# declare-lab/tango

Hardware: NVIDIA H100
Metric: audio_seconds_per_second (higher is better)
Workload: dtype bf16

## Files before the change

tango_b200/csrc/gemm_tc.cu:

```cuda
#include "tng_ptx.cuh"
#include "tng_internal.h"

namespace tng {

constexpr int BM = 128;
constexpr int BK = 64;
constexpr int A_TILE_BYTES = BM * BK * 2;
constexpr int GEMM_THREADS = 384;
constexpr int EPI_WARPS = 8;
constexpr int ES = 4;

struct KGroupDev {
  int view, a_c0, dw, dh, b_k0, nkb;
};

struct GemmKernelParams {
  int W, H, NB;
  int bw, bh, bn;
  int tiles_w, tiles_h, tiles_n;
  int m_tiles, n_tiles;
  int Ncols;
  int n_groups, total_kiters;
  int ksplit;
  KGroupDev g[TNG_MAX_KGROUPS];
  const float* bias;
  const float* rowvec;
  long long rowvec_ld;
  const void* res;
  int res_bf16;
  long long ldr;
  float alpha;
  int accumulate;
  float* out_f32;
  long long ld_f32;
  __nv_bfloat16* out_bf16;
  long long ld_bf16;
  int act;
  float act_param;
  int split_off;
  int fast_epi;
  double* col_stats;
  long long stats_hw;
};

template <int BN>
struct GemmCfg {
  static constexpr int B_TILE_BYTES = BN * BK * 2;
  static constexpr int STAGE_BYTES = A_TILE_BYTES + B_TILE_BYTES;
  static constexpr int EPI_BYTES = EPI_WARPS * 16 * 32 * 4;
  static constexpr int STAGES_RAW = (227 * 1024 - EPI_BYTES - 256) / STAGE_BYTES;
  static constexpr int STAGES = STAGES_RAW > 8 ? 8 : STAGES_RAW;
  static constexpr int SMEM_BYTES = STAGES * STAGE_BYTES + EPI_BYTES + 256 ;
};

enum EpiShape { EPI_SCALAR, EPI_VEC, EPI_FULL };

__device__ __forceinline__ float4 add4(float4 a, float4 b) { return make_float4(a.x + b.x, a.y + b.y, a.z + b.z, a.w + b.w); }
__device__ __forceinline__ float4 scale4(float4 a, float s) { return make_float4(a.x * s, a.y * s, a.z * s, a.w * s); }

template <int ACT>
__device__ __forceinline__ void act_chunk(float4 (&a)[ES], float ap) {
#pragma unroll
  for (int i = 0; i < ES; ++i)
    a[i] = make_float4(act_f(a[i].x, ACT, ap), act_f(a[i].y, ACT, ap), act_f(a[i].z, ACT, ap), act_f(a[i].w, ACT, ap));
}

__device__ __forceinline__ float4 staged(const float* st, int r, int cg) {
  return *reinterpret_cast<const float4*>(st + r * 32 + ((cg ^ (r & 7)) << 2));
}

template <bool VEC, bool RO = false, typename T>
__device__ __forceinline__ float4 load4(const T* q, int n) {
  if constexpr (VEC && sizeof(T) == 2) return load_bf16x4(q);
  if constexpr (VEC && sizeof(T) == 4)
    return RO ? __ldg(reinterpret_cast<const float4*>(q)) : *reinterpret_cast<const float4*>(q);
  float t[4] = {0.f, 0.f, 0.f, 0.f};
#pragma unroll
  for (int j = 0; j < 4; ++j)
    if (j < n) t[j] = static_cast<float>(RO ? __ldg(q + j) : q[j]);
  return make_float4(t[0], t[1], t[2], t[3]);
}

template <bool VEC>
__device__ __forceinline__ float4 load_bias(const GemmKernelParams& p, int col, int n) {
  return p.bias ? load4<VEC, true>(p.bias + col, n) : make_float4(0.f, 0.f, 0.f, 0.f);
}

template <bool VEC>
__device__ __forceinline__ float4 load_res(const GemmKernelParams& p, long long off, int n) {
  return p.res_bf16 ? load4<VEC>(static_cast<const __nv_bfloat16*>(p.res) + off, n)
                    : load4<VEC>(static_cast<const float*>(p.res) + off, n);
}

__device__ __forceinline__ void epi_stage(float* st, int lane, const float* v) {
  const int r = lane >> 2, t = lane & 3;
#pragma unroll
  for (int jj = 0; jj < 4; ++jj) {
    const int col = 8 * jj + 2 * t;
    const int off = (((col >> 2) ^ (r & 7)) << 2) + (col & 3);
    *reinterpret_cast<float2*>(st + r * 32 + off) = make_float2(v[4 * jj], v[4 * jj + 1]);
    *reinterpret_cast<float2*>(st + (r + 8) * 32 + off) = make_float2(v[4 * jj + 2], v[4 * jj + 3]);
  }
}

template <int BN>
__device__ __forceinline__ void stage_chunk(float* st, int lane, const float (&acc)[BN / 2], int c) {
  __syncwarp();
#pragma unroll
  for (int cc = 0; cc < BN / 32; ++cc)
    if (cc == c) epi_stage(st, lane, acc + 16 * cc);
  __syncwarp();
}

struct EpiTile {
  long long row_base;
  int n0, nvalid, tn, sp;
};

template <int BN, int SHAPE, int MODE>
__device__ __forceinline__ void epi_tile(const GemmKernelParams& p, float* st, const float (&acc)[BN / 2], const EpiTile& t,
                                         int wr, int lane) {
  constexpr bool FULL = SHAPE == EPI_FULL, VEC = SHAPE != EPI_SCALAR;
  const int cg = lane & 7, rsub = lane >> 3;
  const int trow = wr + rsub;
  const long long r0 = t.row_base + trow;
  const int lane_rows = FULL ? ES : min(ES, max(0, (t.nvalid - trow + 3) >> 2));
  const bool red = SHAPE == EPI_VEC && p.ksplit > 1;
  const bool add_terms = !red || t.sp == 0;
  const bool has_res = (MODE & 1) && (FULL || p.res) && add_terms;
  const bool has_f32 = (MODE & 2) && (FULL || p.out_f32);
  const bool has_bf = (MODE & 4) && (FULL || p.out_bf16);
  const bool has_rv = p.rowvec && add_terms;
  const int rpi = p.bw * p.bh;
  const int rpi_log2 = __ffs(rpi) - 1;
  const long long simg = (FULL && p.col_stats) ? (t.row_base + wr) / p.stats_hw : 0;
  const float4 zero = make_float4(0.f, 0.f, 0.f, 0.f);
#pragma unroll 1
  for (int c = 0; c < BN / 32; ++c) {
    stage_chunk<BN>(st, lane, acc, c);
    const int col = t.tn * BN + 32 * c + 4 * cg;
    const int ncols = FULL ? 4 : min(4, p.Ncols - col);
    const int nrows = ncols > 0 ? lane_rows : 0;
    float4 res[ES];
    if (has_res) {
      const long long off = r0 * p.ldr + col, rs = 4 * p.ldr;
#pragma unroll
      for (int i = 0; i < ES; ++i) res[i] = i < nrows ? load_res<VEC>(p, off + i * rs, ncols) : zero;
    }
    const float4 b4 = (add_terms && ncols > 0) ? load_bias<VEC>(p, col, ncols) : zero;
    float4 a[ES];
#pragma unroll
    for (int i = 0; i < ES; ++i) a[i] = add4(staged(st, 4 * i + rsub, cg), b4);
    if (has_rv) {
      float4 rv = zero;
#pragma unroll
      for (int i = 0; i < ES; ++i) {
        if (i >= nrows) continue;
        const long long img = t.n0 + ((trow + 4 * i) >> rpi_log2);
        if (i == 0 || rpi % 16 != 0) rv = load4<VEC, true>(p.rowvec + img * p.rowvec_ld + col, ncols);
        a[i] = add4(a[i], rv);
      }
    }
#pragma unroll
    for (int i = 0; i < ES; ++i) a[i] = scale4(has_res ? add4(a[i], res[i]) : a[i], p.alpha);
    if (has_f32) {
      float* op = p.out_f32 + r0 * p.ld_f32 + col;
      const long long os = 4 * p.ld_f32;
      if (p.accumulate) {
#pragma unroll
        for (int i = 0; i < ES; ++i)
          if (i < nrows) a[i] = add4(a[i], load4<VEC>(op + i * os, ncols));
      }
#pragma unroll
      for (int i = 0; i < ES; ++i) {
        if (i >= nrows) continue;
        float* q = op + i * os;
        if (red) {
          atomicAdd(q, a[i].x); atomicAdd(q + 1, a[i].y); atomicAdd(q + 2, a[i].z); atomicAdd(q + 3, a[i].w);
        } else if (VEC) {
          *reinterpret_cast<float4*>(q) = a[i];
        } else {
          const float v[4] = {a[i].x, a[i].y, a[i].z, a[i].w};
#pragma unroll
          for (int j = 0; j < 4; ++j)
            if (j < ncols) q[j] = v[j];
        }
      }
    }
    if (FULL && p.col_stats) {
      float s0 = 0.f, s1 = 0.f, s2 = 0.f, s3 = 0.f, q0 = 0.f, q1 = 0.f, q2 = 0.f, q3 = 0.f;
#pragma unroll
      for (int i = 0; i < ES; ++i) {
        s0 += a[i].x; s1 += a[i].y; s2 += a[i].z; s3 += a[i].w;
        q0 = fmaf(a[i].x, a[i].x, q0); q1 = fmaf(a[i].y, a[i].y, q1);
        q2 = fmaf(a[i].z, a[i].z, q2); q3 = fmaf(a[i].w, a[i].w, q3);
      }
#pragma unroll
      for (int o = 8; o <= 16; o <<= 1) {
        s0 += __shfl_xor_sync(0xffffffffu, s0, o); s1 += __shfl_xor_sync(0xffffffffu, s1, o);
        s2 += __shfl_xor_sync(0xffffffffu, s2, o); s3 += __shfl_xor_sync(0xffffffffu, s3, o);
        q0 += __shfl_xor_sync(0xffffffffu, q0, o); q1 += __shfl_xor_sync(0xffffffffu, q1, o);
        q2 += __shfl_xor_sync(0xffffffffu, q2, o); q3 += __shfl_xor_sync(0xffffffffu, q3, o);
      }
      if (rsub == 0) {
        double* sp = p.col_stats + (simg * p.Ncols + col) * 2;
        atomicAdd(sp + 0, static_cast<double>(s0)); atomicAdd(sp + 1, static_cast<double>(q0));
        atomicAdd(sp + 2, static_cast<double>(s1)); atomicAdd(sp + 3, static_cast<double>(q1));
        atomicAdd(sp + 4, static_cast<double>(s2)); atomicAdd(sp + 5, static_cast<double>(q2));
        atomicAdd(sp + 6, static_cast<double>(s3)); atomicAdd(sp + 7, static_cast<double>(q3));
      }
    }
    if (has_bf) {
      if (p.act == TNG_ACT_SILU) act_chunk<TNG_ACT_SILU>(a, p.act_param);
      else if (p.act == TNG_ACT_LRELU) act_chunk<TNG_ACT_LRELU>(a, p.act_param);
      __nv_bfloat16* op = p.out_bf16 + r0 * p.ld_bf16 + col;
      const long long os = 4 * p.ld_bf16;
#pragma unroll
      for (int i = 0; i < ES; ++i) {
        if (i >= nrows) continue;
        if (VEC) {
          store4_bf16(op + i * os, a[i]);
        } else {
          const float v[4] = {a[i].x, a[i].y, a[i].z, a[i].w};
#pragma unroll
          for (int j = 0; j < 4; ++j)
            if (j < ncols) store_bf16_split(op + i * os + j, v[j], p.split_off);
        }
      }
      if (VEC && p.split_off > 0) {
#pragma unroll
        for (int i = 0; i < ES; ++i)
          if (i < nrows) store4_bf16_lo(op + p.split_off + i * os, a[i]);
      }
    }
  }
}

template <int BN, bool FULL, bool SPLIT, bool TANH>
__device__ __forceinline__ void epi_tile_geglu(const GemmKernelParams& p, float* st, const float (&acc)[BN / 2],
                                               const EpiTile& t, int wr, int lane) {
  constexpr int HALF = BN / 2;
  const int cg = lane & 7, rsub = lane >> 3;
  const int trow = wr + rsub;
#pragma unroll 1
  for (int c = 0; c < HALF / 32; ++c) {
    float4 hid[ES], g[ES];
    stage_chunk<BN>(st, lane, acc, c);
#pragma unroll
    for (int i = 0; i < ES; ++i) hid[i] = staged(st, 4 * i + rsub, cg);
    stage_chunk<BN>(st, lane, acc, c + HALF / 32);
#pragma unroll
    for (int i = 0; i < ES; ++i) g[i] = staged(st, 4 * i + rsub, cg);
    const int gcol = t.tn * BN + 32 * c + 4 * cg;
    const int ocol = t.tn * HALF + 32 * c + 4 * cg;
    const float4 bh = load_bias<true>(p, gcol, 4), bg = load_bias<true>(p, gcol + HALF, 4);
#pragma unroll
    for (int i = 0; i < ES; ++i) {
      hid[i].x = (hid[i].x + bh.x) * (TANH ? gelu_tanh_f(g[i].x + bg.x) : gelu_erf_f(g[i].x + bg.x));
      hid[i].y = (hid[i].y + bh.y) * (TANH ? gelu_tanh_f(g[i].y + bg.y) : gelu_erf_f(g[i].y + bg.y));
      hid[i].z = (hid[i].z + bh.z) * (TANH ? gelu_tanh_f(g[i].z + bg.z) : gelu_erf_f(g[i].z + bg.z));
      hid[i].w = (hid[i].w + bh.w) * (TANH ? gelu_tanh_f(g[i].w + bg.w) : gelu_erf_f(g[i].w + bg.w));
    }
    __nv_bfloat16* op = p.out_bf16 + (t.row_base + trow) * p.ld_bf16 + ocol;
    const long long os = 4 * p.ld_bf16;
#pragma unroll
    for (int i = 0; i < ES; ++i) {
      if (!FULL && trow + 4 * i >= t.nvalid) continue;
      store4_bf16(op + i * os, hid[i]);
      if (SPLIT) store4_bf16_lo(op + p.split_off + i * os, hid[i]);
    }
  }
}

struct WorkItem {
  int sp, tn, w0, h0, n0;
};
__device__ __forceinline__ WorkItem work_item(const GemmKernelParams& p, int tile) {
  const int t2 = tile / p.ksplit, tm = t2 / p.n_tiles;
  const int tw = tm % p.tiles_w, th = (tm / p.tiles_w) % p.tiles_h, tb = tm / (p.tiles_w * p.tiles_h);
  return WorkItem{tile % p.ksplit, t2 % p.n_tiles, tw * p.bw, th * p.bh, tb * p.bn};
}

__device__ __forceinline__ int tile_kiters(const GemmKernelParams& p, int tile) {
  const int sp = tile % p.ksplit;
  return (sp + 1) * p.total_kiters / p.ksplit - sp * p.total_kiters / p.ksplit;
}

template <int BN>
__global__ void __launch_bounds__(GEMM_THREADS, 1)
gemm_tc_kernel(const __grid_constant__ CUtensorMap amap0, const __grid_constant__ CUtensorMap amap1,
               const __grid_constant__ CUtensorMap amap2, const __grid_constant__ CUtensorMap amap3,
               const __grid_constant__ CUtensorMap bmap, const __grid_constant__ GemmKernelParams p) {
  using Cfg = GemmCfg<BN>;
  constexpr int STAGES = Cfg::STAGES;
  extern __shared__ __align__(1024) uint8_t smem[];
  uint8_t* sA = smem;
  uint8_t* sB = smem + STAGES * A_TILE_BYTES;
  float* sEpi = reinterpret_cast<float*>(smem + STAGES * Cfg::STAGE_BYTES);
  uint64_t* full_bar = reinterpret_cast<uint64_t*>(smem + STAGES * Cfg::STAGE_BYTES + Cfg::EPI_BYTES);
  uint64_t* empty_bar = full_bar + STAGES;

  const int tid = threadIdx.x;
  const int warp = tid >> 5;
  const int lane = tid & 31;
  const int wg = warp >> 2;

  if (tid == 0) {
    if ((smem_u32(smem) & 1023u) != 0) __trap();
    tma_prefetch_desc(&amap0);
    tma_prefetch_desc(&bmap);
    for (int s = 0; s < STAGES; ++s) {
      mbar_init(&full_bar[s], 1);
      mbar_init(&empty_bar[s], 2);
    }
    fence_mbar_init();
  }
  __syncthreads();

  const int total_tiles = p.m_tiles * p.n_tiles * p.ksplit;
  const int work0 = blockIdx.x, work_stride = gridDim.x;

  if (wg == 0) {
    setmaxnreg_dec<40>();
    if (tid == 0) {
      uint32_t n_loaded = 0;
      for (int tile = work0; tile < total_tiles; tile += work_stride) {
        const WorkItem w = work_item(p, tile);
        const int nk = tile_kiters(p, tile);
        int k = w.sp * p.total_kiters / p.ksplit, gi = 0;
        while (k >= p.g[gi].nkb) { k -= p.g[gi].nkb; ++gi; }
        for (int ki = 0; ki < nk; ++ki, ++k, ++n_loaded) {
          if (k == p.g[gi].nkb) { k = 0; ++gi; }
          const int slot = static_cast<int>(n_loaded % STAGES);
          const uint32_t use = n_loaded / STAGES;
          if (use > 0) mbar_wait(&empty_bar[slot], (use - 1) & 1);
          const KGroupDev g = p.g[gi];
          const CUtensorMap* am = g.view == 0 ? &amap0 : g.view == 1 ? &amap1 : g.view == 2 ? &amap2 : &amap3;
          mbar_arrive_expect_tx(&full_bar[slot], Cfg::STAGE_BYTES);
          tma_load_4d(sA + slot * A_TILE_BYTES, am, &full_bar[slot], g.a_c0 + k * BK, w.w0 + g.dw, w.h0 + g.dh, w.n0);
          tma_load_2d(sB + slot * Cfg::B_TILE_BYTES, &bmap, &full_bar[slot], g.b_k0 + k * BK, w.tn * BN);
        }
      }
    }
    return;
  }
  setmaxnreg_inc<232>();

  const int cw = warp - 4;
  float* st = sEpi + cw * (16 * 32);
  const int wr = 16 * cw;
  const uint32_t a_off = static_cast<uint32_t>(wg - 1) * (64 * 128);
  const bool release = (tid & 127) == 0;
  const int mode = (p.res ? 1 : 0) | (p.out_f32 ? 2 : 0) | (p.out_bf16 ? 4 : 0);
  const bool geglu = (p.act == TNG_ACT_GEGLU || p.act == TNG_ACT_GEGLU_TANH);
  uint32_t n_used = 0;
  float acc[BN / 2];
#pragma unroll
  for (int i = 0; i < BN / 2; ++i) acc[i] = 0.f;
  for (int tile = work0; tile < total_tiles; tile += work_stride) {
    const int nk = tile_kiters(p, tile);
    for (int ki = 0; ki < nk; ++ki) {
      const int slot = static_cast<int>(n_used % STAGES);
      mbar_wait(&full_bar[slot], (n_used / STAGES) & 1);
      const uint64_t ad = wgmma_desc_sw128(smem_u32(sA + slot * A_TILE_BYTES) + a_off, 16, 1024);
      const uint64_t bd = wgmma_desc_sw128(smem_u32(sB + slot * Cfg::B_TILE_BYTES), 16, 1024);
      fence_regs(acc);
      wgmma_fence();
#pragma unroll
      for (int k = 0; k < BK / 16; ++k) wgmma_ss<BN>(acc, ad + 2 * k, bd + 2 * k, (ki > 0 || k > 0) ? 1u : 0u);
      wgmma_commit();
      fence_regs(acc);
      if (ki > 0) {
        wgmma_wait<1>();
        fence_regs(acc);
        mbar_arrive_if(&empty_bar[(n_used - 1) % STAGES], release);
      }
      ++n_used;
    }
    wgmma_wait<0>();
    fence_regs(acc);
    mbar_arrive_if(&empty_bar[(n_used - 1) % STAGES], release);

    const WorkItem w = work_item(p, tile);
    int nvalid;
    if (p.bh == 1 && p.bn == 1) nvalid = min(BM, p.W - w.w0);
    else if (p.bn == 1) nvalid = min(p.bh, p.H - w.h0) * p.bw;
    else nvalid = min(p.bn, p.NB - w.n0) * p.bh * p.bw;
    const EpiTile t{(static_cast<long long>(w.n0) * p.H + w.h0) * p.W + w.w0, w.n0, nvalid, w.tn, w.sp};
    if (geglu) {
      if constexpr (BN == 128 || BN == 256) {
        if (p.act == TNG_ACT_GEGLU_TANH) {
          if (p.split_off > 0) epi_tile_geglu<BN, false, true, true>(p, st, acc, t, wr, lane);
          else epi_tile_geglu<BN, false, false, true>(p, st, acc, t, wr, lane);
        } else if (p.split_off > 0) epi_tile_geglu<BN, false, true, false>(p, st, acc, t, wr, lane);
        else if (nvalid == BM) epi_tile_geglu<BN, true, false, false>(p, st, acc, t, wr, lane);
        else epi_tile_geglu<BN, false, false, false>(p, st, acc, t, wr, lane);
      }
    } else if (p.fast_epi && p.ksplit == 1 && nvalid == BM && (w.tn + 1) * BN <= p.Ncols) {
      switch (mode) {
        case 2: epi_tile<BN, EPI_FULL, 2>(p, st, acc, t, wr, lane); break;
        case 3: epi_tile<BN, EPI_FULL, 3>(p, st, acc, t, wr, lane); break;
        case 4: epi_tile<BN, EPI_FULL, 4>(p, st, acc, t, wr, lane); break;
        case 5: epi_tile<BN, EPI_FULL, 5>(p, st, acc, t, wr, lane); break;
        case 6: epi_tile<BN, EPI_FULL, 6>(p, st, acc, t, wr, lane); break;
        default: epi_tile<BN, EPI_FULL, 7>(p, st, acc, t, wr, lane); break;
      }
    } else if (p.fast_epi) {
      epi_tile<BN, EPI_VEC, 7>(p, st, acc, t, wr, lane);
    } else {
      epi_tile<BN, EPI_SCALAR, 7>(p, st, acc, t, wr, lane);
    }
  }
}

template <int BN>
static int launch_gemm(const CUtensorMap* am, const CUtensorMap& bm, const GemmKernelParams& p, cudaStream_t st) {
  using Cfg = GemmCfg<BN>;
  const int rc = set_max_dynamic_smem<gemm_tc_kernel<BN>>(Cfg::SMEM_BYTES, "gemm_tc");
  if (rc) return rc;
  const int work = p.m_tiles * p.n_tiles * p.ksplit;
  const int grid = work < num_sms() ? work : num_sms();
  gemm_tc_kernel<BN><<<grid, GEMM_THREADS, Cfg::SMEM_BYTES, st>>>(am[0], am[1], am[2], am[3], bm, p);
  return check_launch("gemm_tc");
}

static bool is_pow2(long long x) { return x > 0 && (x & (x - 1)) == 0; }

}

using namespace tng;

static int plan_gemm(const tng_gemm_desc* d, GemmKernelParams& p, int& bn_tile_out, bool& stats_after_out) {
  if (!d) return set_error(TNG_EINVAL, "null desc");
  if (d->n_aviews < 1 || d->n_aviews > TNG_MAX_AVIEWS) return set_error(TNG_EINVAL, "n_aviews=%d", d->n_aviews);
  if (d->n_groups < 1 || d->n_groups > TNG_MAX_KGROUPS) return set_error(TNG_EINVAL, "n_groups=%d", d->n_groups);
  if (d->W <= 0 || d->H <= 0 || d->NB <= 0 || d->Ncols <= 0) return set_error(TNG_EINVAL, "bad output grid");
  if ((d->ldb > 0 ? d->ldb : d->Ktot) % 8 != 0)
    return set_error(TNG_EINVAL, "B row stride must be a multiple of 8 elements (Ktot=%lld ldb=%lld)", (long long)d->Ktot, (long long)d->ldb);

  memset(&p, 0, sizeof(p));
  p.W = d->W; p.H = d->H; p.NB = d->NB;
  if (d->W >= BM || d->H == 1) {
    p.bw = BM; p.bh = 1; p.bn = 1;
  } else {
    if (!is_pow2(d->W)) return set_error(TNG_EINVAL, "W=%d < 128 must be a power of two", d->W);
    p.bw = d->W;
    const int rem = BM / p.bw;
    if (d->H >= rem) {
      p.bh = rem; p.bn = 1;
    } else {
      if (!is_pow2(d->H)) return set_error(TNG_EINVAL, "H=%d (W=%d) must be a power of two when W*H < 128", d->H, d->W);
      p.bh = d->H; p.bn = rem / p.bh;
    }
  }
  p.tiles_w = (d->W + p.bw - 1) / p.bw;
  p.tiles_h = (d->H + p.bh - 1) / p.bh;
  p.tiles_n = (d->NB + p.bn - 1) / p.bn;
  p.m_tiles = p.tiles_w * p.tiles_h * p.tiles_n;
  p.Ncols = (int)d->Ncols;

  int bn_tile = d->block_n;
  int ksplit = 1;
  if (d->act == TNG_ACT_GEGLU || d->act == TNG_ACT_GEGLU_TANH) {
    if (bn_tile == 0) bn_tile = (d->Ncols % 256 == 0) ? 256 : 128;
    if ((bn_tile != 128 && bn_tile != 256) || d->Ncols % bn_tile != 0 || !d->out_bf16 || d->out_f32 || d->res ||
        d->rowvec)
      return set_error(TNG_EINVAL, "GEGLU epilogue needs block_n 128/256 dividing Ncols, bf16 output only");
    if (d->alpha != 1.0f) return set_error(TNG_EINVAL, "GEGLU epilogue needs alpha = 1 (alpha=%g)", (double)d->alpha);
  }
  if (bn_tile == 0) {
    const long long N = d->Ncols;
    if (N <= 32) bn_tile = 32;
    else if (N <= 64) bn_tile = 64;
    else if (N % 256 == 0 && (long long)p.m_tiles * (N / 256) >= 2 * num_sms()) bn_tile = 256;
    else if (N % 160 == 0) {
      bn_tile = 160;
      if ((long long)p.m_tiles * (N / 160) * 2 <= num_sms()) {
        long long kit = 0;
        for (int i = 0; i < d->n_groups; ++i) kit += d->g[i].nkb;
        const bool can_split = d->out_f32 && !d->out_bf16 && !d->accumulate && d->act == TNG_ACT_NONE &&
                               d->res != d->out_f32 && kit >= 32 && d->Ncols % 4 == 0;
        if (can_split) ksplit = 2;
        else if (N % 128 == 0 && (long long)p.m_tiles * (N / 128) <= num_sms()) bn_tile = 128;
      }
    }
    else if (N % 128 == 0) bn_tile = 128;
    else if (N % 64 == 0 && N < 256) bn_tile = 64;
    else bn_tile = 128;
  }
  p.n_tiles = (int)((d->Ncols + bn_tile - 1) / bn_tile);
  p.ksplit = ksplit;

  p.n_groups = d->n_groups;
  p.total_kiters = 0;
  for (int i = 0; i < d->n_groups; ++i) {
    const tng_kgroup& g = d->g[i];
    if (g.view < 0 || g.view >= d->n_aviews || g.nkb <= 0) return set_error(TNG_EINVAL, "k-group %d invalid", i);
    if (g.b_k0 < 0 || g.b_k0 + (long long)(g.nkb - 1) * BK >= d->Ktot)
      return set_error(TNG_EINVAL, "k-group %d: K block outside B", i);
    if (g.a_c0 < 0 || g.a_c0 + (long long)(g.nkb - 1) * BK >= d->a[g.view].C)
      return set_error(TNG_EINVAL, "k-group %d: K block outside view channels", i);
    p.g[i] = KGroupDev{g.view, g.a_c0, g.dw, g.dh, g.b_k0, g.nkb};
    p.total_kiters += g.nkb;
  }
  p.bias = d->bias; p.rowvec = d->rowvec; p.rowvec_ld = d->rowvec_ld > 0 ? d->rowvec_ld : d->Ncols; p.res = d->res; p.res_bf16 = (d->res_dtype == TNG_DT_BF16);
  p.ldr = d->ldr; p.alpha = d->alpha; p.accumulate = d->accumulate;
  p.out_f32 = d->out_f32; p.ld_f32 = d->ld_f32;
  p.out_bf16 = reinterpret_cast<__nv_bfloat16*>(d->out_bf16); p.ld_bf16 = d->ld_bf16;
  p.act = d->act; p.act_param = d->act_param; p.split_off = d->split_off;
  if (!d->out_f32 && !d->out_bf16) return set_error(TNG_EINVAL, "no output");
  if (d->accumulate && !d->out_f32) return set_error(TNG_EINVAL, "accumulate needs out_f32");

  auto al16 = [](const void* q) { return (reinterpret_cast<uintptr_t>(q) & 15) == 0; };
  bool vec = true;
  if (d->bias && !al16(d->bias)) vec = false;
  if (d->rowvec && (!al16(d->rowvec) || p.rowvec_ld % 4)) vec = false;
  if (d->res) {
    if (!al16(d->res)) vec = false;
    if (p.res_bf16 ? (d->ldr % 8) : (d->ldr % 4)) vec = false;
  }
  if (d->out_f32 && (!al16(d->out_f32) || d->ld_f32 % 4)) vec = false;
  if (d->out_bf16 && (!al16(d->out_bf16) || d->ld_bf16 % 8 || d->split_off % 8)) vec = false;
  p.fast_epi = (vec && d->Ncols % 4 == 0) ? 1 : 0;
  if ((d->act == TNG_ACT_GEGLU || d->act == TNG_ACT_GEGLU_TANH) && !vec) return set_error(TNG_EINVAL, "GEGLU epilogue needs 16-byte aligned output");
  if (d->gn_stats) {
    if (d->stats_hw <= 0 || (static_cast<long long>(d->W) * d->H * d->NB) % d->stats_hw != 0)
      return set_error(TNG_EINVAL, "gn_stats: the output rows must be whole images of stats_hw pixels");
    if (!d->out_f32 && (d->split_off > 0 || d->act != TNG_ACT_NONE))
      return set_error(TNG_EINVAL, "gn_stats without an fp32 output needs a plain bf16 output (no activation, no hi/lo split)");
  }

  const bool full_m = (p.bh == 1 && p.bn == 1) ? (d->W % BM == 0) : (p.bn == 1 ? (d->H % p.bh == 0) : (d->NB % p.bn == 0));
  if (p.ksplit > 1 && !p.fast_epi) p.ksplit = 1;
  bool stats_after = false;
  if (d->gn_stats) {
    const bool fused = full_m && (d->Ncols % bn_tile == 0) && p.fast_epi && p.ksplit == 1 && !d->accumulate &&
                       (d->stats_hw % 16 == 0) && d->act != TNG_ACT_GEGLU && d->act != TNG_ACT_GEGLU_TANH;
    if (fused) { p.col_stats = d->gn_stats; p.stats_hw = d->stats_hw; }
    else stats_after = true;
  }
  bn_tile_out = bn_tile;
  stats_after_out = stats_after;
  return TNG_OK;
}

extern "C" int tng_gemm_plan(const tng_gemm_desc* d, int32_t* block_n, int32_t* mode, int32_t* ksplit) {
  GemmKernelParams p;
  int bn_tile = 0;
  bool stats_after = false;
  const int rc = plan_gemm(d, p, bn_tile, stats_after);
  if (rc != TNG_OK) return rc;
  if (block_n) *block_n = bn_tile;
  if (mode) *mode = 1;
  if (ksplit) *ksplit = p.ksplit;
  return TNG_OK;
}

extern "C" int tng_conv_gemm(const tng_gemm_desc* d, void* stream) {
  GemmKernelParams p;
  int bn_tile = 0;
  bool stats_after = false;
  {
    const int rc = plan_gemm(d, p, bn_tile, stats_after);
    if (rc != TNG_OK) return rc;
  }
  CUtensorMap am[4];
  for (int i = 0; i < 4; ++i) {
    const tng_aview& v = d->a[i < d->n_aviews ? i : 0];
    if (v.C % 8 != 0) return set_error(TNG_EINVAL, "view %d: C=%lld must be a multiple of 8", i, (long long)v.C);
    uint64_t dims[4] = {(uint64_t)v.C, (uint64_t)v.W, (uint64_t)v.H, (uint64_t)v.NB};
    uint64_t strides[3] = {(uint64_t)v.s_w * 2, (uint64_t)v.s_h * 2, (uint64_t)v.s_n * 2};
    uint32_t box[4] = {(uint32_t)BK, (uint32_t)p.bw, (uint32_t)p.bh, (uint32_t)p.bn};
    int rc = encode_tmap_bf16(&am[i], v.ptr, 4, dims, strides, box);
    if (rc) return rc;
  }
  CUtensorMap bm;
  {
    uint64_t dims[2] = {(uint64_t)d->Ktot, (uint64_t)d->Ncols};
    uint64_t strides[1] = {(uint64_t)(d->ldb > 0 ? d->ldb : d->Ktot) * 2};
    uint32_t box[2] = {(uint32_t)BK, (uint32_t)bn_tile};
    int rc = encode_tmap_bf16(&bm, d->b, 2, dims, strides, box);
    if (rc) return rc;
  }
  cudaStream_t st = reinterpret_cast<cudaStream_t>(stream);
  if (p.ksplit > 1) {
    const size_t rows = static_cast<size_t>(d->W) * d->H * d->NB;
    cudaError_t e = cudaMemset2DAsync(d->out_f32, static_cast<size_t>(d->ld_f32) * 4, 0, static_cast<size_t>(d->Ncols) * 4, rows, st);
    if (e != cudaSuccess) return set_error(TNG_ECUDA, "cudaMemset2DAsync(split-K output): %s", cudaGetErrorString(e));
  }
  int rc;
  switch (bn_tile) {
    case 32: rc = launch_gemm<32>(am, bm, p, st); break;
    case 64: rc = launch_gemm<64>(am, bm, p, st); break;
    case 128: rc = launch_gemm<128>(am, bm, p, st); break;
    case 160: rc = launch_gemm<160>(am, bm, p, st); break;
    case 256: rc = launch_gemm<256>(am, bm, p, st); break;
    default: return set_error(TNG_EINVAL, "block_n=%d unsupported", bn_tile);
  }
  if (rc == TNG_OK && stats_after) {
    const long long rows = static_cast<long long>(d->W) * d->H * d->NB;
    if (d->out_f32) rc = launch_col_stats(d->out_f32, TNG_DT_F32, d->Ncols, d->ld_f32, rows / d->stats_hw, d->stats_hw, d->gn_stats, st);
    else rc = launch_col_stats(d->out_bf16, TNG_DT_BF16, d->Ncols, d->ld_bf16, rows / d->stats_hw, d->stats_hw, d->gn_stats, st);
  }
  return rc;
}
```

Before: 12.60.

## Add ping-pong consumer warpgroup schedule for narrow and GEGLU GEMM tiles

For BN<=64, and for BN=128 with GEGLU, each consumer warpgroup now computes all 128 rows of alternating tiles instead of splitting one tile's rows. An order barrier serializes the two warpgroups' mainloops, so one warpgroup's epilogue can overlap the other's MMA loop. The kernel takes a GEGLU template flag so the dispatch is fixed at compile time, and empty barriers expect one arrival in ping mode. The cost is a doubled accumulator register footprint for those tile sizes, and two extra mbarriers placed after the existing ones, which must fit in the allocated shared memory.

```diff
diff --git a/tango_b200/csrc/gemm_tc.cu b/tango_b200/csrc/gemm_tc.cu
--- a/tango_b200/csrc/gemm_tc.cu
+++ b/tango_b200/csrc/gemm_tc.cu
@@ -286,19 +286,22 @@
   return (sp + 1) * p.total_kiters / p.ksplit - sp * p.total_kiters / p.ksplit;
 }
 
-template <int BN>
+template <int BN, bool GEGLU>
 __global__ void __launch_bounds__(GEMM_THREADS, 1)
 gemm_tc_kernel(const __grid_constant__ CUtensorMap amap0, const __grid_constant__ CUtensorMap amap1,
                const __grid_constant__ CUtensorMap amap2, const __grid_constant__ CUtensorMap amap3,
                const __grid_constant__ CUtensorMap bmap, const __grid_constant__ GemmKernelParams p) {
   using Cfg = GemmCfg<BN>;
   constexpr int STAGES = Cfg::STAGES;
+  constexpr bool PING = BN <= 64 || (BN == 128 && GEGLU);
+  constexpr int MH = PING ? 2 : 1;
   extern __shared__ __align__(1024) uint8_t smem[];
   uint8_t* sA = smem;
   uint8_t* sB = smem + STAGES * A_TILE_BYTES;
   float* sEpi = reinterpret_cast<float*>(smem + STAGES * Cfg::STAGE_BYTES);
   uint64_t* full_bar = reinterpret_cast<uint64_t*>(smem + STAGES * Cfg::STAGE_BYTES + Cfg::EPI_BYTES);
   uint64_t* empty_bar = full_bar + STAGES;
+  uint64_t* order_bar = empty_bar + STAGES;
 
   const int tid = threadIdx.x;
   const int warp = tid >> 5;
@@ -311,8 +314,10 @@
     tma_prefetch_desc(&bmap);
     for (int s = 0; s < STAGES; ++s) {
       mbar_init(&full_bar[s], 1);
-      mbar_init(&empty_bar[s], 2);
-    }
+      mbar_init(&empty_bar[s], PING ? 1 : 2);
+    }
+    mbar_init(&order_bar[0], 1);
+    mbar_init(&order_bar[1], 1);
     fence_mbar_init();
   }
   __syncthreads();
@@ -346,39 +351,59 @@
   }
   setmaxnreg_inc<232>();
 
+  const int c = wg - 1;
   const int cw = warp - 4;
   float* st = sEpi + cw * (16 * 32);
-  const int wr = 16 * cw;
-  const uint32_t a_off = static_cast<uint32_t>(wg - 1) * (64 * 128);
   const bool release = (tid & 127) == 0;
   const int mode = (p.res ? 1 : 0) | (p.out_f32 ? 2 : 0) | (p.out_bf16 ? 4 : 0);
-  const bool geglu = (p.act == TNG_ACT_GEGLU || p.act == TNG_ACT_GEGLU_TANH);
   uint32_t n_used = 0;
-  float acc[BN / 2];
-#pragma unroll
-  for (int i = 0; i < BN / 2; ++i) acc[i] = 0.f;
+  float acc[MH][BN / 2];
+#pragma unroll
+  for (int h = 0; h < MH; ++h)
+#pragma unroll
+    for (int i = 0; i < BN / 2; ++i) acc[h][i] = 0.f;
   for (int tile = work0; tile < total_tiles; tile += work_stride) {
     const int nk = tile_kiters(p, tile);
+    if (PING) {
+      const int item = (tile - work0) / work_stride;
+      if ((item & 1) != c) {
+        n_used += nk;
+        continue;
+      }
+      if (item > 0) mbar_wait(&order_bar[c], ((item - 1) >> 1) & 1);
+    }
     for (int ki = 0; ki < nk; ++ki) {
       const int slot = static_cast<int>(n_used % STAGES);
       mbar_wait(&full_bar[slot], (n_used / STAGES) & 1);
-      const uint64_t ad = wgmma_desc_sw128(smem_u32(sA + slot * A_TILE_BYTES) + a_off, 16, 1024);
+      const uint32_t a_base = smem_u32(sA + slot * A_TILE_BYTES);
       const uint64_t bd = wgmma_desc_sw128(smem_u32(sB + slot * Cfg::B_TILE_BYTES), 16, 1024);
-      fence_regs(acc);
+#pragma unroll
+      for (int h = 0; h < MH; ++h) fence_regs(acc[h]);
       wgmma_fence();
 #pragma unroll
-      for (int k = 0; k < BK / 16; ++k) wgmma_ss<BN>(acc, ad + 2 * k, bd + 2 * k, (ki > 0 || k > 0) ? 1u : 0u);
+      for (int k = 0; k < BK / 16; ++k) {
+#pragma unroll
+        for (int h = 0; h < MH; ++h) {
+          const uint32_t a_off = static_cast<uint32_t>(PING ? h : c) * (64 * 128);
+          const uint64_t ad = wgmma_desc_sw128(a_base + a_off, 16, 1024);
+          wgmma_ss<BN>(acc[h], ad + 2 * k, bd + 2 * k, (ki > 0 || k > 0) ? 1u : 0u);
+        }
+      }
       wgmma_commit();
-      fence_regs(acc);
+#pragma unroll
+      for (int h = 0; h < MH; ++h) fence_regs(acc[h]);
       if (ki > 0) {
         wgmma_wait<1>();
-        fence_regs(acc);
+#pragma unroll
+        for (int h = 0; h < MH; ++h) fence_regs(acc[h]);
         mbar_arrive_if(&empty_bar[(n_used - 1) % STAGES], release);
       }
       ++n_used;
     }
+    if (PING) mbar_arrive_if(&order_bar[c ^ 1], release);
     wgmma_wait<0>();
-    fence_regs(acc);
+#pragma unroll
+    for (int h = 0; h < MH; ++h) fence_regs(acc[h]);
     mbar_arrive_if(&empty_bar[(n_used - 1) % STAGES], release);
 
     const WorkItem w = work_item(p, tile);
@@ -387,40 +412,44 @@
     else if (p.bn == 1) nvalid = min(p.bh, p.H - w.h0) * p.bw;
     else nvalid = min(p.bn, p.NB - w.n0) * p.bh * p.bw;
     const EpiTile t{(static_cast<long long>(w.n0) * p.H + w.h0) * p.W + w.w0, w.n0, nvalid, w.tn, w.sp};
-    if (geglu) {
-      if constexpr (BN == 128 || BN == 256) {
-        if (p.act == TNG_ACT_GEGLU_TANH) {
-          if (p.split_off > 0) epi_tile_geglu<BN, false, true, true>(p, st, acc, t, wr, lane);
-          else epi_tile_geglu<BN, false, false, true>(p, st, acc, t, wr, lane);
-        } else if (p.split_off > 0) epi_tile_geglu<BN, false, true, false>(p, st, acc, t, wr, lane);
-        else if (nvalid == BM) epi_tile_geglu<BN, true, false, false>(p, st, acc, t, wr, lane);
-        else epi_tile_geglu<BN, false, false, false>(p, st, acc, t, wr, lane);
-      }
-    } else if (p.fast_epi && p.ksplit == 1 && nvalid == BM && (w.tn + 1) * BN <= p.Ncols) {
-      switch (mode) {
-        case 2: epi_tile<BN, EPI_FULL, 2>(p, st, acc, t, wr, lane); break;
-        case 3: epi_tile<BN, EPI_FULL, 3>(p, st, acc, t, wr, lane); break;
-        case 4: epi_tile<BN, EPI_FULL, 4>(p, st, acc, t, wr, lane); break;
-        case 5: epi_tile<BN, EPI_FULL, 5>(p, st, acc, t, wr, lane); break;
-        case 6: epi_tile<BN, EPI_FULL, 6>(p, st, acc, t, wr, lane); break;
-        default: epi_tile<BN, EPI_FULL, 7>(p, st, acc, t, wr, lane); break;
-      }
-    } else if (p.fast_epi) {
-      epi_tile<BN, EPI_VEC, 7>(p, st, acc, t, wr, lane);
-    } else {
-      epi_tile<BN, EPI_SCALAR, 7>(p, st, acc, t, wr, lane);
-    }
-  }
-}
-
-template <int BN>
+#pragma unroll
+    for (int h = 0; h < MH; ++h) {
+      const int wr = 64 * (PING ? h : c) + 16 * (cw & 3);
+      if constexpr (GEGLU) {
+        if constexpr (BN == 128 || BN == 256) {
+          if (p.act == TNG_ACT_GEGLU_TANH) {
+            if (p.split_off > 0) epi_tile_geglu<BN, false, true, true>(p, st, acc[h], t, wr, lane);
+            else epi_tile_geglu<BN, false, false, true>(p, st, acc[h], t, wr, lane);
+          } else if (p.split_off > 0) epi_tile_geglu<BN, false, true, false>(p, st, acc[h], t, wr, lane);
+          else if (nvalid == BM) epi_tile_geglu<BN, true, false, false>(p, st, acc[h], t, wr, lane);
+          else epi_tile_geglu<BN, false, false, false>(p, st, acc[h], t, wr, lane);
+        }
+      } else if (p.fast_epi && p.ksplit == 1 && nvalid == BM && (w.tn + 1) * BN <= p.Ncols) {
+        switch (mode) {
+          case 2: epi_tile<BN, EPI_FULL, 2>(p, st, acc[h], t, wr, lane); break;
+          case 3: epi_tile<BN, EPI_FULL, 3>(p, st, acc[h], t, wr, lane); break;
+          case 4: epi_tile<BN, EPI_FULL, 4>(p, st, acc[h], t, wr, lane); break;
+          case 5: epi_tile<BN, EPI_FULL, 5>(p, st, acc[h], t, wr, lane); break;
+          case 6: epi_tile<BN, EPI_FULL, 6>(p, st, acc[h], t, wr, lane); break;
+          default: epi_tile<BN, EPI_FULL, 7>(p, st, acc[h], t, wr, lane); break;
+        }
+      } else if (p.fast_epi) {
+        epi_tile<BN, EPI_VEC, 7>(p, st, acc[h], t, wr, lane);
+      } else {
+        epi_tile<BN, EPI_SCALAR, 7>(p, st, acc[h], t, wr, lane);
+      }
+    }
+  }
+}
+
+template <int BN, bool GEGLU>
 static int launch_gemm(const CUtensorMap* am, const CUtensorMap& bm, const GemmKernelParams& p, cudaStream_t st) {
   using Cfg = GemmCfg<BN>;
-  const int rc = set_max_dynamic_smem<gemm_tc_kernel<BN>>(Cfg::SMEM_BYTES, "gemm_tc");
+  const int rc = set_max_dynamic_smem<gemm_tc_kernel<BN, GEGLU>>(Cfg::SMEM_BYTES, "gemm_tc");
   if (rc) return rc;
   const int work = p.m_tiles * p.n_tiles * p.ksplit;
   const int grid = work < num_sms() ? work : num_sms();
-  gemm_tc_kernel<BN><<<grid, GEMM_THREADS, Cfg::SMEM_BYTES, st>>>(am[0], am[1], am[2], am[3], bm, p);
+  gemm_tc_kernel<BN, GEGLU><<<grid, GEMM_THREADS, Cfg::SMEM_BYTES, st>>>(am[0], am[1], am[2], am[3], bm, p);
   return check_launch("gemm_tc");
 }
 
@@ -589,13 +618,17 @@
     if (e != cudaSuccess) return set_error(TNG_ECUDA, "cudaMemset2DAsync(split-K output): %s", cudaGetErrorString(e));
   }
   int rc;
-  switch (bn_tile) {
-    case 32: rc = launch_gemm<32>(am, bm, p, st); break;
-    case 64: rc = launch_gemm<64>(am, bm, p, st); break;
-    case 128: rc = launch_gemm<128>(am, bm, p, st); break;
-    case 160: rc = launch_gemm<160>(am, bm, p, st); break;
-    case 256: rc = launch_gemm<256>(am, bm, p, st); break;
-    default: return set_error(TNG_EINVAL, "block_n=%d unsupported", bn_tile);
+  if (d->act == TNG_ACT_GEGLU || d->act == TNG_ACT_GEGLU_TANH) {
+    rc = bn_tile == 128 ? launch_gemm<128, true>(am, bm, p, st) : launch_gemm<256, true>(am, bm, p, st);
+  } else {
+    switch (bn_tile) {
+      case 32: rc = launch_gemm<32, false>(am, bm, p, st); break;
+      case 64: rc = launch_gemm<64, false>(am, bm, p, st); break;
+      case 128: rc = launch_gemm<128, false>(am, bm, p, st); break;
+      case 160: rc = launch_gemm<160, false>(am, bm, p, st); break;
+      case 256: rc = launch_gemm<256, false>(am, bm, p, st); break;
+      default: return set_error(TNG_EINVAL, "block_n=%d unsupported", bn_tile);
+    }
   }
   if (rc == TNG_OK && stats_after) {
     const long long rows = static_cast<long long>(d->W) * d->H * d->NB;
```

After: 12.62 (median of 6 runs). Within noise of the previous version (+0.1%).
